# nv-tlabs/LION

Measured on AMD Instinct MI355X. Metric: shapes/sec @1000-step DDIM, Bx2048pts, higher is better.
Workload: dtype f32 (operands of the 3x3x3 voxel convolutions and of the long 1x1 convolutions cut into fp16 hi/lo pairs on the 16-bi...

## Files before the change

lion_amd/csrc/conv3d_split.hip:

```cpp
#include "conv3d_split_kernel.h"

namespace {

__global__ void split_pack_kernel(const float *__restrict__ w, int Cout, int Cin, unsigned short *__restrict__ wp,
                                  unsigned *__restrict__ tail) {
  const int i = blockIdx.x * blockDim.x + threadIdx.x;
  const int ew = split_tail_scale(tail, i == 0);
  if (i >= Cout * Cin * 27) return;
  const int t = i % 27, c = (i / 27) % Cin, co = i / (27 * Cin), chunk = c / KS, g = (c % KS) / 8, j = c % 8;
  unsigned short hi, lo;
  cut(w[i] * pow2f(ew), hi, lo);
  const size_t base = ((size_t)chunk * 27 + t) * 4;
  wp[((base + 0 + g) * Cout + co) * 8 + j] = hi;
  wp[((base + 2 + g) * Cout + co) * 8 + j] = lo;
}

template <bool PRO, bool STATS, int NW>
__global__ __launch_bounds__(64 * NW, 1) void conv3d_split_pipe_kernel(const float *__restrict__ x, const u4 *__restrict__ wp,
                                                                  const float *__restrict__ wtail,
                                                                  const float *__restrict__ bias, float *__restrict__ y,
                                                                  int Cin, int Cout, const float *__restrict__ pro_a,
                                                                  const float *__restrict__ pro_b,
                                                                  float *__restrict__ stats) {
  constexpr int r = 8, r3 = 512, TD = 4, TH = 8, TW = 8, VB = 8 / NW, COT = 32, TM = 64 * NW;
  static_assert(NW == 4 || NW == 8, "4 waves x 2 column blocks or 8 waves x 1");
  constexpr int HD = TD + 2, HH = TH + 2, HW = NW == 8 ? TW + 4 : TW + 2, HALO = HD * HH * HW;
  constexpr int HP = (HALO + 63) / 64 * 64;
  constexpr int WPL = 4 * COT, TG = 9, NG = 27 / TG;
  constexpr int DMA_PER_GROUP = TG * WPL / 64, DMA_MIN = DMA_PER_GROUP / NW;
  extern __shared__ __attribute__((aligned(16))) unsigned char smem[];
  u4 *sx = reinterpret_cast<u4 *>(smem);
  u4 *sw = sx + 2 * 4 * HP;
  float *sbias = reinterpret_cast<float *>(sw + 3 * TG * WPL);
  const int npro = PRO ? ((Cin + 63) & ~63) : 0;
  float *spa = sbias + COT, *spb = spa + npro;
  float *sred = spb + npro;
  __shared__ unsigned s_max[2];
  const int tid = threadIdx.x, lane = tid & 63, wave = __builtin_amdgcn_readfirstlane(tid >> 6);
  const int g = lane >> 5, l32 = lane & 31;
  const int b = blockIdx.x, tile = blockIdx.y, co0 = blockIdx.z * COT, d0 = tile * TD;
  const float wscale_inv = wtail[2];
  if (PRO)
    for (int c = tid; c < Cin; c += TM) { spa[c] = pro_a[(size_t)b * Cin + c]; spb[c] = pro_b[(size_t)b * Cin + c]; }
  if (tid < COT) sbias[tid] = bias ? bias[co0 + tid] : 0.f;
  if (tid < 2) s_max[tid] = 0u;
  int E = 127;

  static_assert(NW == 8, "the quad staging is laid out for 512 threads");
  constexpr int NLOAD = 4;
  const int st_ig = tid / 192, st_u = tid % 192, st_ch4 = st_u / 96, st_rq = st_u % 96;
  const int st_row = st_rq >> 1, st_quad = st_rq & 1, st_hd = st_row >> 3, st_gh = st_row & 7;
  const int st_gd = d0 - 1 + st_hd;
  const bool gok = tid < 384 && st_gd >= 0 && st_gd < r;
  const int goff = gok ? ((st_gd * r + st_gh) * r + st_quad * 4) * 4 + (st_ig * 8 + st_ch4 * 4) * r3 * 4 : 0x7fffff00;
  const int st_pos = (st_hd * HH + st_gh + 1) * HW + st_quad * 4 + 1;
  const __amdgpu_buffer_rsrc_t xrs = __builtin_amdgcn_make_buffer_rsrc(
      const_cast<float *>(x + (size_t)b * Cin * r3), 0, Cin * r3 * 4, 0x00020000);
  int xbase[VB], vox[VB];
#pragma unroll
  for (int vb = 0; vb < VB; ++vb) {
    const int vbk = wave * VB + vb;
    const int d = vbk >> 1, w = l32 & 7;
    const int h = NW == 8 ? (vbk & 1) + 2 * (l32 >> 3) : (vbk & 1) * 2 + ((l32 >> 4) & 1) + 4 * ((l32 >> 3) & 1);
    xbase[vb] = (d * HH + h) * HW + w;
    vox[vb] = ((d0 + d) * r + h) * r + w;
  }
  f32x16 acc[VB], cor[VB], cor2[VB];
#pragma unroll
  for (int vb = 0; vb < VB; ++vb)
#pragma unroll
    for (int i = 0; i < 16; ++i) acc[vb][i] = cor[vb][i] = cor2[vb][i] = 0.f;

  const int nchunks = Cin / KS, ngroups = nchunks * NG;
  typedef __attribute__((address_space(3))) unsigned char lds_byte;
  const uint32_t sw_lds = (uint32_t)(uintptr_t)(lds_byte *)reinterpret_cast<unsigned char *>(sw);
  auto weights_dma = [&](int sg) {
    const u4 *src = wp + (size_t)sg * TG * 4 * Cout + co0;
    const uint32_t dst0 = sw_lds + (uint32_t)((sg % 3) * TG * WPL * 16);
    for (int i = wave; i < DMA_PER_GROUP; i += NW) {
      const u4 *gp = src + (size_t)((i >> 1) * 4 + (i & 1) * 2 + g) * Cout + l32;
      const uint32_t dst = __builtin_amdgcn_readfirstlane(dst0 + (uint32_t)(i * 1024));
      unsigned keep;
      asm volatile("s_mov_b32 %0, m0\n\ts_mov_b32 m0, %2\n\ts_nop 0\n\tglobal_load_lds_dwordx4 %1, off\n\ts_mov_b32 m0, %0"
                   : "=&s"(keep) : "v"(gp), "s"(dst) : "memory");
    }
  };
  typedef float f4 __attribute__((ext_vector_type(4)));
  f4 v[NLOAD];
  auto issue_loads = [&](int q) {
#pragma unroll
    for (int j = 0; j < NLOAD; ++j)
      v[j] = __builtin_bit_cast(f4, __builtin_amdgcn_raw_buffer_load_b128(xrs, goff, (q * KS + j) * r3 * 4, 0));
  };
  auto stage = [&](int q) {
    unsigned mloc = 0u;
    if (PRO) {
      const int c0 = q * KS + st_ig * 8 + st_ch4 * 4;
      const float4 a4 = *reinterpret_cast<const float4 *>(spa + (tid < 384 ? c0 : 0));
      const float4 b4 = *reinterpret_cast<const float4 *>(spb + (tid < 384 ? c0 : 0));
      const float pa[4] = {a4.x, a4.y, a4.z, a4.w}, pb[4] = {b4.x, b4.y, b4.z, b4.w};
#pragma unroll
      for (int j = 0; j < NLOAD; ++j)
#pragma unroll
        for (int k = 0; k < 4; ++k) {
          const float act = pro_act(v[j][k], pa[j], pb[j]);
          v[j][k] = gok ? act : 0.f;
        }
    }
#pragma unroll
    for (int j = 0; j < NLOAD; ++j)
#pragma unroll
      for (int k = 0; k < 4; ++k) {
        const unsigned a = __float_as_uint(v[j][k]) & 0x7fffffffu;
        mloc = (a > mloc && a <= 0x7f7fffffu) ? a : mloc;
      }
    mloc = wave_max_u32_lane63(mloc);
    if (lane == 63 && mloc) atomicMax(&s_max[q & 1], mloc);
    __syncthreads();
    const unsigned mbits = s_max[q & 1];
    if (tid == 0) s_max[(q + 1) & 1] = 0u;
    if (mbits) {
      const int e = scale_exp(__uint_as_float(mbits));
      if (e < E) {
        if (E != 127) {
          const float f = pow2f(max(e - CONV_SPLIT_HEADROOM - E, -126));
#pragma unroll
          for (int vb = 0; vb < VB; ++vb)
#pragma unroll
            for (int i = 0; i < 16; ++i) { acc[vb][i] *= f; cor[vb][i] *= f; cor2[vb][i] *= f; }
        }
        E = e - CONV_SPLIT_HEADROOM;
      }
    }
    const float xs = E == 127 ? 1.0f : pow2f(E);
    if (tid < 384) {
      uint2 *dst2 = reinterpret_cast<uint2 *>(sx + (q & 1) * 4 * HP);
#pragma unroll
      for (int k = 0; k < 4; ++k) {
        unsigned h0, l0, h1, l1;
        cut2(v[0][k] * xs, v[1][k] * xs, h0, l0);
        cut2(v[2][k] * xs, v[3][k] * xs, h1, l1);
        dst2[((0 + st_ig) * HP + st_pos + k) * 2 + st_ch4] = make_uint2(h0, h1);
        dst2[((2 + st_ig) * HP + st_pos + k) * 2 + st_ch4] = make_uint2(l0, l1);
      }
    }
  };

  for (int e = tid; e < 2 * 4 * HP; e += TM) sx[e] = u4{0u, 0u, 0u, 0u};
  weights_dma(0);
  if (ngroups > 1) weights_dma(1);
  issue_loads(0);
  __syncthreads();
  stage(0);
  for (int q = 0; q < nchunks; ++q) {
    const u4 *sxq = sx + (q & 1) * 4 * HP;
    const bool more = q + 1 < nchunks;
#pragma unroll
    for (int grp = 0; grp < NG; ++grp) {
      const int sg = q * NG + grp;
      const bool dma_behind = sg + 1 < ngroups;
      if (grp == 0 || !more) { if (dma_behind) wait_vm<DMA_MIN>(); else wait_vm<0>(); }
      else { if (dma_behind) wait_vm<DMA_MIN + NLOAD>(); else wait_vm<NLOAD>(); }
      __syncthreads();
      if (sg + 2 < ngroups) weights_dma(sg + 2);
      if (grp == 0 && more) issue_loads(q + 1);
      const u4 *swg = sw + (sg % 3) * TG * WPL;
      u4 wf[2][2], xf[2][VB][2];
      auto frags = [&](int t, int s_) {
        const int tap = grp * TG + t;
        const int toff = ((tap / 9) * HH + (tap / 3) % 3) * HW + tap % 3;
#pragma unroll
        for (int pc = 0; pc < 2; ++pc) {
          wf[s_][pc] = swg[t * WPL + (pc * 2 + g) * COT + l32];
#pragma unroll
          for (int vb = 0; vb < VB; ++vb) xf[s_][vb][pc] = sxq[(pc * 2 + g) * HP + xbase[vb] + toff];
        }
      };
      frags(0, 0);
#pragma unroll
      for (int t = 0; t < TG; ++t) {
        if (t + 1 < TG) frags(t + 1, (t + 1) & 1);
        __builtin_amdgcn_sched_barrier(0);
#pragma unroll
        for (int vb = 0; vb < VB; ++vb) {
          acc[vb] = mma(wf[t & 1][0], xf[t & 1][vb][0], acc[vb]);
          cor[vb] = mma(wf[t & 1][0], xf[t & 1][vb][1], cor[vb]);
          cor2[vb] = mma(wf[t & 1][1], xf[t & 1][vb][0], cor2[vb]);
        }
        __builtin_amdgcn_sched_barrier(0);
      }
    }
    if (more) stage(q + 1);
  }

  float *yb = y + ((size_t)b * Cout + co0) * r3;
  const float us_x = E == 127 ? 1.0f : pow2f(-E), us_w = wscale_inv;
#pragma unroll
  for (int vb = 0; vb < VB; ++vb)
#pragma unroll
    for (int i = 0; i < 16; ++i) {
      const int co = (i & 3) + 8 * (i >> 2) + 4 * g;
      const float o = ((acc[vb][i] + (cor[vb][i] + cor2[vb][i]) * (1.f / 2048.f)) * us_x) * us_w + sbias[co];
      acc[vb][i] = o;
      yb[(size_t)co * r3 + vox[vb]] = o;
    }
  if (STATS) {
#pragma unroll
    for (int i = 0; i < 16; ++i) {
      float s1 = acc[0][i], s2 = acc[0][i] * acc[0][i];
#pragma unroll
      for (int vb = 1; vb < VB; ++vb) { s1 += acc[vb][i]; s2 += acc[vb][i] * acc[vb][i]; }
      s1 = row16_sum_rn(s1); s2 = row16_sum_rn(s2);
      s1 = row_pair_sum_odd_rows(s1); s2 = row_pair_sum_odd_rows(s2);
      if (l32 == 16) {
        const int co = (i & 3) + 8 * (i >> 2) + 4 * g;
        sred[(wave * COT + co) * 2] = s1;
        sred[(wave * COT + co) * 2 + 1] = s2;
      }
    }
    __syncthreads();
    if (tid < COT) {
      float s1 = 0.f, s2 = 0.f;
#pragma unroll
      for (int w = 0; w < NW; ++w) { s1 += sred[(w * COT + tid) * 2]; s2 += sred[(w * COT + tid) * 2 + 1]; }
      float *o = stats + (((size_t)b * Cout + co0 + tid) * (r / TD) + tile) * 2;
      o[0] = s1;
      o[1] = s2;
    }
  }
}

template <int NW>
static int launch_split_pipe(const float *x, const u4 *wp, const float *wtail, const float *bias, float *y, int B, int Cin,
                             int Cout, const float *pa, const float *pb, float *stats, hipStream_t st) {
  constexpr int HP = NW == 8 ? 768 : 640, COT = 32;
  const dim3 grid(B, 2, Cout / COT);
  const size_t LDS = (size_t)(2 * 4 * HP + 3 * 9 * 4 * COT) * 16 +
                     (size_t)(COT + (pa ? 2 * ((Cin + 63) & ~63) : 0) + NW * COT * 2) * 4;
#define LION_PIPE_GO(PRO_, ST_)                                                                              \
  {                                                                                                          \
    static LionLdsLimit cfg = {};                                                                            \
    if (int e = lion_dynamic_lds(&conv3d_split_pipe_kernel<PRO_, ST_, NW>, LDS, cfg)) return e;              \
    conv3d_split_pipe_kernel<PRO_, ST_, NW><<<grid, 64 * NW, LDS, st>>>(x, wp, wtail, bias, y, Cin, Cout, pa, pb, stats); \
  }
  if (pa && stats) LION_PIPE_GO(true, true)
  else if (pa) LION_PIPE_GO(true, false)
  else if (stats) LION_PIPE_GO(false, true)
  else LION_PIPE_GO(false, false)
#undef LION_PIPE_GO
  LION_LAUNCH_CHECK();
  return 0;
}

struct SplitPlan { int vb, cb, tiles; };
static SplitPlan split_plan(int r, int Cout) {
  const int r3 = r * r * r;
  const int cb = Cout % 64 == 0 ? 2 : Cout % 32 == 0 ? 1 : 0;
  if (r == 8) return {2, Cout % 32 == 0 ? 1 : 0, 2};
  return {2, cb, r3 / 256};
}

}

extern "C" {

size_t lion_conv3d_split_packed_halfs(int Cout, int Cin) { return split_piece_halfs(Cout, Cin) + 8; }

int lion_conv3d_split_pack_weights(const float *w, int Cout, int Cin, uint16_t *wp, lionStream_t stream) {
  if (!w || !wp || Cout <= 0 || Cin <= 0) return LION_EINVAL;
  if (Cin % KS != 0 || (((uintptr_t)wp) & 15) != 0) return LION_EUNSUPPORTED;
  hipStream_t st = static_cast<hipStream_t>(stream);
  unsigned *tail = reinterpret_cast<unsigned *>(wp + split_piece_halfs(Cout, Cin));
  const int n = Cout * Cin * 27;
  if (hipMemsetAsync(tail, 0, 16, st) != hipSuccess) return LION_EINVAL;
  split_wmax_kernel<<<min(lion_cdiv(n, 2048), 128), 256, 0, st>>>(w, n, tail);
  split_pack_kernel<<<lion_cdiv(n, 256), 256, 0, st>>>(w, Cout, Cin, wp, tail);
  LION_LAUNCH_CHECK();
  return 0;
}


int lion_conv3d_split_stat_tiles(int r, int Cout) {
  if (r != 8 && r != 16 && r != 32) return 0;
  return split_plan(r, Cout).tiles;
}

int lion_conv3d_k3_split_forward(const float *x, const uint16_t *wp, const float *bias, int B, int Cin, int Cout,
                                 int r, const float *pro_a, const float *pro_b, const float *pro_bias,
                                 const float *tconst, float *y, float *stats, int32_t *occ, lionStream_t stream) {
  if (!x || !wp || !y || B <= 0 || Cin <= 0 || Cout <= 0) return LION_EINVAL;
  if ((pro_a == nullptr) != (pro_b == nullptr)) return LION_EINVAL;
  if (tconst && !pro_a) return LION_EINVAL;
  if (occ && pro_a && !tconst) return LION_EINVAL;
  if (Cin % KS != 0 || (pro_a && Cin > 256)) return LION_EUNSUPPORTED;
  if (r != 8 && r != 16 && r != 32) return LION_EUNSUPPORTED;
  if (occ && r == 8) return LION_EUNSUPPORTED;
  const SplitPlan p = split_plan(r, Cout);
  if (!p.cb) return LION_EUNSUPPORTED;
  hipStream_t st = static_cast<hipStream_t>(stream);
  const u4 *w4 = reinterpret_cast<const u4 *>(wp);
  const float *wtail = reinterpret_cast<const float *>(wp + split_piece_halfs(Cout, Cin));
  if (r == 8) {
    if (tconst) return LION_EUNSUPPORTED;
    return launch_split_pipe<8>(x, w4, wtail, bias, y, B, Cin, Cout, pro_a, pro_b, stats, st);
  }
#define LION_SPLIT_TILE(R_, VB_, CB_, TD_, TH_, TW_, OCC_)                                                  \
  if (r == R_ && p.vb == VB_ && p.cb == CB_)                                                                \
    return launch_split_t<TD_, TH_, TW_, CB_, VB_, OCC_, 2>(x, w4, wtail, bias, y, B, Cin, Cout, r, pro_a, pro_b, pro_bias, tconst, \
                                                   stats, occ, st);
  LION_SPLIT_TILE(32, 2, 2, 2, 4, 32, 2)
  LION_SPLIT_TILE(32, 2, 1, 2, 4, 32, 2)
  LION_SPLIT_TILE(16, 2, 2, 4, 4, 16, 2)
  LION_SPLIT_TILE(16, 2, 1, 4, 4, 16, 2)
#undef LION_SPLIT_TILE
  return LION_EUNSUPPORTED;
}

}
```

Baseline: 5.378.

## Interleave next-chunk staging into r=8 conv MMA loop behind env toggle

Adds an OVL template mode to the r=8 voxel conv pipeline kernel. The next chunk's activation, max reduction, rescale and hi/lo cut-and-store are sliced across the tap loop of the current chunk's MMA groups, so they no longer run as a serial stage between chunks. The initial DMA and loads are also issued before the LDS zero-fill. The NW template is removed and the kernel is hardwired to 8 waves. The mode is on by default and can be disabled with LION_CONV_R8_OVERLAP=0. It risks extra register pressure and schedule interference with the MMA stream, and the s_max reset timing changes.

```diff
diff --git a/lion_amd/csrc/conv3d_split.hip b/lion_amd/csrc/conv3d_split.hip
--- a/lion_amd/csrc/conv3d_split.hip
+++ b/lion_amd/csrc/conv3d_split.hip
@@ -15,16 +15,15 @@
   wp[((base + 2 + g) * Cout + co) * 8 + j] = lo;
 }
 
-template <bool PRO, bool STATS, int NW>
-__global__ __launch_bounds__(64 * NW, 1) void conv3d_split_pipe_kernel(const float *__restrict__ x, const u4 *__restrict__ wp,
-                                                                  const float *__restrict__ wtail,
-                                                                  const float *__restrict__ bias, float *__restrict__ y,
-                                                                  int Cin, int Cout, const float *__restrict__ pro_a,
-                                                                  const float *__restrict__ pro_b,
-                                                                  float *__restrict__ stats) {
-  constexpr int r = 8, r3 = 512, TD = 4, TH = 8, TW = 8, VB = 8 / NW, COT = 32, TM = 64 * NW;
-  static_assert(NW == 4 || NW == 8, "4 waves x 2 column blocks or 8 waves x 1");
-  constexpr int HD = TD + 2, HH = TH + 2, HW = NW == 8 ? TW + 4 : TW + 2, HALO = HD * HH * HW;
+template <bool PRO, bool STATS, bool OVL>
+__global__ __launch_bounds__(512, 1) void conv3d_split_pipe_kernel(const float *__restrict__ x, const u4 *__restrict__ wp,
+                                                                 const float *__restrict__ wtail,
+                                                                 const float *__restrict__ bias, float *__restrict__ y,
+                                                                 int Cin, int Cout, const float *__restrict__ pro_a,
+                                                                 const float *__restrict__ pro_b,
+                                                                 float *__restrict__ stats) {
+  constexpr int NW = 8, r = 8, r3 = 512, TD = 4, TH = 8, TW = 8, COT = 32, TM = 64 * NW;
+  constexpr int HD = TD + 2, HH = TH + 2, HW = TW + 4, HALO = HD * HH * HW;
   constexpr int HP = (HALO + 63) / 64 * 64;
   constexpr int WPL = 4 * COT, TG = 9, NG = 27 / TG;
   constexpr int DMA_PER_GROUP = TG * WPL / 64, DMA_MIN = DMA_PER_GROUP / NW;
@@ -46,7 +45,6 @@
   if (tid < 2) s_max[tid] = 0u;
   int E = 127;
 
-  static_assert(NW == 8, "the quad staging is laid out for 512 threads");
   constexpr int NLOAD = 4;
   const int st_ig = tid / 192, st_u = tid % 192, st_ch4 = st_u / 96, st_rq = st_u % 96;
   const int st_row = st_rq >> 1, st_quad = st_rq & 1, st_hd = st_row >> 3, st_gh = st_row & 7;
@@ -56,20 +54,11 @@
   const int st_pos = (st_hd * HH + st_gh + 1) * HW + st_quad * 4 + 1;
   const __amdgpu_buffer_rsrc_t xrs = __builtin_amdgcn_make_buffer_rsrc(
       const_cast<float *>(x + (size_t)b * Cin * r3), 0, Cin * r3 * 4, 0x00020000);
-  int xbase[VB], vox[VB];
-#pragma unroll
-  for (int vb = 0; vb < VB; ++vb) {
-    const int vbk = wave * VB + vb;
-    const int d = vbk >> 1, w = l32 & 7;
-    const int h = NW == 8 ? (vbk & 1) + 2 * (l32 >> 3) : (vbk & 1) * 2 + ((l32 >> 4) & 1) + 4 * ((l32 >> 3) & 1);
-    xbase[vb] = (d * HH + h) * HW + w;
-    vox[vb] = ((d0 + d) * r + h) * r + w;
-  }
-  f32x16 acc[VB], cor[VB], cor2[VB];
-#pragma unroll
-  for (int vb = 0; vb < VB; ++vb)
-#pragma unroll
-    for (int i = 0; i < 16; ++i) acc[vb][i] = cor[vb][i] = cor2[vb][i] = 0.f;
+  const int vd = wave >> 1, vw = l32 & 7, vh = (wave & 1) + 2 * (l32 >> 3);
+  const int xbase = (vd * HH + vh) * HW + vw, vox = ((d0 + vd) * r + vh) * r + vw;
+  f32x16 acc, cor, cor2;
+#pragma unroll
+  for (int i = 0; i < 16; ++i) acc[i] = cor[i] = cor2[i] = 0.f;
 
   const int nchunks = Cin / KS, ngroups = nchunks * NG;
   typedef __attribute__((address_space(3))) unsigned char lds_byte;
@@ -92,69 +81,97 @@
     for (int j = 0; j < NLOAD; ++j)
       v[j] = __builtin_bit_cast(f4, __builtin_amdgcn_raw_buffer_load_b128(xrs, goff, (q * KS + j) * r3 * 4, 0));
   };
+  float pa[NLOAD], pb[NLOAD];
+  auto pro_scalars = [&](int q) {
+    const int c0 = q * KS + st_ig * 8 + st_ch4 * 4;
+    const float4 a4 = *reinterpret_cast<const float4 *>(spa + (tid < 384 ? c0 : 0));
+    const float4 b4 = *reinterpret_cast<const float4 *>(spb + (tid < 384 ? c0 : 0));
+    pa[0] = a4.x; pa[1] = a4.y; pa[2] = a4.z; pa[3] = a4.w;
+    pb[0] = b4.x; pb[1] = b4.y; pb[2] = b4.z; pb[3] = b4.w;
+  };
+  auto activate = [&](int j, int k) {
+    const float act = pro_act(v[j][k], pa[j], pb[j]);
+    v[j][k] = gok ? act : 0.f;
+  };
+  auto finite_max = [&](unsigned m, int j, int k) {
+    const unsigned a = __float_as_uint(v[j][k]) & 0x7fffffffu;
+    return (a > m && a <= 0x7f7fffffu) ? a : m;
+  };
+  auto publish_max = [&](unsigned m, int q) {
+    m = wave_max_u32_lane63(m);
+    if (lane == 63 && m) atomicMax(&s_max[q & 1], m);
+  };
+  auto next_scale = [&](unsigned mbits) {
+    if (mbits) {
+      const int e = scale_exp(__uint_as_float(mbits));
+      if (e < E) return e - CONV_SPLIT_HEADROOM;
+    }
+    return E;
+  };
+  auto rescale_to = [&](int En) {
+    if (En != E) {
+      if (E != 127) {
+        const float f = pow2f(max(En - E, -126));
+#pragma unroll
+        for (int i = 0; i < 16; ++i) { acc[i] *= f; cor[i] *= f; cor2[i] *= f; }
+      }
+      E = En;
+    }
+  };
+  auto cut_store = [&](int q, int k, float xs) {
+    if (tid < 384) {
+      uint2 *dst2 = reinterpret_cast<uint2 *>(sx + (q & 1) * 4 * HP);
+      unsigned h0, l0, h1, l1;
+      cut2(v[0][k] * xs, v[1][k] * xs, h0, l0);
+      cut2(v[2][k] * xs, v[3][k] * xs, h1, l1);
+      dst2[((0 + st_ig) * HP + st_pos + k) * 2 + st_ch4] = make_uint2(h0, h1);
+      dst2[((2 + st_ig) * HP + st_pos + k) * 2 + st_ch4] = make_uint2(l0, l1);
+    }
+  };
   auto stage = [&](int q) {
     unsigned mloc = 0u;
     if (PRO) {
-      const int c0 = q * KS + st_ig * 8 + st_ch4 * 4;
-      const float4 a4 = *reinterpret_cast<const float4 *>(spa + (tid < 384 ? c0 : 0));
-      const float4 b4 = *reinterpret_cast<const float4 *>(spb + (tid < 384 ? c0 : 0));
-      const float pa[4] = {a4.x, a4.y, a4.z, a4.w}, pb[4] = {b4.x, b4.y, b4.z, b4.w};
+      pro_scalars(q);
 #pragma unroll
       for (int j = 0; j < NLOAD; ++j)
 #pragma unroll
-        for (int k = 0; k < 4; ++k) {
-          const float act = pro_act(v[j][k], pa[j], pb[j]);
-          v[j][k] = gok ? act : 0.f;
-        }
+        for (int k = 0; k < 4; ++k) activate(j, k);
     }
 #pragma unroll
     for (int j = 0; j < NLOAD; ++j)
 #pragma unroll
-      for (int k = 0; k < 4; ++k) {
-        const unsigned a = __float_as_uint(v[j][k]) & 0x7fffffffu;
-        mloc = (a > mloc && a <= 0x7f7fffffu) ? a : mloc;
-      }
-    mloc = wave_max_u32_lane63(mloc);
-    if (lane == 63 && mloc) atomicMax(&s_max[q & 1], mloc);
+      for (int k = 0; k < 4; ++k) mloc = finite_max(mloc, j, k);
+    publish_max(mloc, q);
     __syncthreads();
     const unsigned mbits = s_max[q & 1];
-    if (tid == 0) s_max[(q + 1) & 1] = 0u;
-    if (mbits) {
-      const int e = scale_exp(__uint_as_float(mbits));
-      if (e < E) {
-        if (E != 127) {
-          const float f = pow2f(max(e - CONV_SPLIT_HEADROOM - E, -126));
-#pragma unroll
-          for (int vb = 0; vb < VB; ++vb)
-#pragma unroll
-            for (int i = 0; i < 16; ++i) { acc[vb][i] *= f; cor[vb][i] *= f; cor2[vb][i] *= f; }
-        }
-        E = e - CONV_SPLIT_HEADROOM;
-      }
-    }
+    if (!OVL && tid == 0) s_max[(q + 1) & 1] = 0u;
+    rescale_to(next_scale(mbits));
     const float xs = E == 127 ? 1.0f : pow2f(E);
-    if (tid < 384) {
-      uint2 *dst2 = reinterpret_cast<uint2 *>(sx + (q & 1) * 4 * HP);
-#pragma unroll
-      for (int k = 0; k < 4; ++k) {
-        unsigned h0, l0, h1, l1;
-        cut2(v[0][k] * xs, v[1][k] * xs, h0, l0);
-        cut2(v[2][k] * xs, v[3][k] * xs, h1, l1);
-        dst2[((0 + st_ig) * HP + st_pos + k) * 2 + st_ch4] = make_uint2(h0, h1);
-        dst2[((2 + st_ig) * HP + st_pos + k) * 2 + st_ch4] = make_uint2(l0, l1);
-      }
-    }
-  };
-
+#pragma unroll
+    for (int k = 0; k < 4; ++k) cut_store(q, k, xs);
+  };
+
+  if (OVL) {
+    weights_dma(0);
+    if (ngroups > 1) weights_dma(1);
+    issue_loads(0);
+  }
   for (int e = tid; e < 2 * 4 * HP; e += TM) sx[e] = u4{0u, 0u, 0u, 0u};
-  weights_dma(0);
-  if (ngroups > 1) weights_dma(1);
-  issue_loads(0);
+  if (!OVL) {
+    weights_dma(0);
+    if (ngroups > 1) weights_dma(1);
+    issue_loads(0);
+  }
   __syncthreads();
+  if (OVL) __builtin_amdgcn_sched_barrier(0);
   stage(0);
-  for (int q = 0; q < nchunks; ++q) {
+  auto chunk = [&](int q, auto more_c) {
+    constexpr bool SLICE = OVL && decltype(more_c)::value;
+    const bool more = OVL ? SLICE : q + 1 < nchunks;
     const u4 *sxq = sx + (q & 1) * 4 * HP;
-    const bool more = q + 1 < nchunks;
+    unsigned mloc = 0u;
+    int E_next = E;
+    float xs_next = 1.0f;
 #pragma unroll
     for (int grp = 0; grp < NG; ++grp) {
       const int sg = q * NG + grp;
@@ -162,54 +179,82 @@
       if (grp == 0 || !more) { if (dma_behind) wait_vm<DMA_MIN>(); else wait_vm<0>(); }
       else { if (dma_behind) wait_vm<DMA_MIN + NLOAD>(); else wait_vm<NLOAD>(); }
       __syncthreads();
+      if (OVL && grp == 0 && tid == 0) s_max[q & 1] = 0u;
       if (sg + 2 < ngroups) weights_dma(sg + 2);
       if (grp == 0 && more) issue_loads(q + 1);
+      if (SLICE) {
+        if (PRO && grp == 1) pro_scalars(q + 1);
+        if (grp == 2) {
+          E_next = next_scale(s_max[(q + 1) & 1]);
+          xs_next = E_next == 127 ? 1.0f : pow2f(E_next);
+        }
+      }
       const u4 *swg = sw + (sg % 3) * TG * WPL;
-      u4 wf[2][2], xf[2][VB][2];
+      u4 wf[2][2], xf[2][2];
       auto frags = [&](int t, int s_) {
         const int tap = grp * TG + t;
         const int toff = ((tap / 9) * HH + (tap / 3) % 3) * HW + tap % 3;
 #pragma unroll
         for (int pc = 0; pc < 2; ++pc) {
           wf[s_][pc] = swg[t * WPL + (pc * 2 + g) * COT + l32];
-#pragma unroll
-          for (int vb = 0; vb < VB; ++vb) xf[s_][vb][pc] = sxq[(pc * 2 + g) * HP + xbase[vb] + toff];
+          xf[s_][pc] = sxq[(pc * 2 + g) * HP + xbase + toff];
         }
       };
       frags(0, 0);
 #pragma unroll
       for (int t = 0; t < TG; ++t) {
+        if (SLICE && grp == 1 && t == 1) wait_vm<DMA_MIN>();
         if (t + 1 < TG) frags(t + 1, (t + 1) & 1);
+        auto slice = [&]() {
+          if (grp == 1 && t >= 1) {
+#pragma unroll
+            for (int i = 2 * (t - 1); i < 2 * t; ++i) {
+              if (PRO) activate(i >> 2, i & 3);
+              mloc = finite_max(mloc, i >> 2, i & 3);
+            }
+          }
+          if (grp == 2 && (t & 1)) cut_store(q + 1, t >> 1, xs_next);
+        };
+        if (SLICE) slice();
         __builtin_amdgcn_sched_barrier(0);
-#pragma unroll
-        for (int vb = 0; vb < VB; ++vb) {
-          acc[vb] = mma(wf[t & 1][0], xf[t & 1][vb][0], acc[vb]);
-          cor[vb] = mma(wf[t & 1][0], xf[t & 1][vb][1], cor[vb]);
-          cor2[vb] = mma(wf[t & 1][1], xf[t & 1][vb][0], cor2[vb]);
+        acc = mma(wf[t & 1][0], xf[t & 1][0], acc);
+        cor = mma(wf[t & 1][0], xf[t & 1][1], cor);
+        cor2 = mma(wf[t & 1][1], xf[t & 1][0], cor2);
+        __builtin_amdgcn_sched_barrier(0);
+      }
+      if (SLICE) {
+        if (grp == 1) {
+          publish_max(mloc, q + 1);
         }
-        __builtin_amdgcn_sched_barrier(0);
-      }
-    }
-    if (more) stage(q + 1);
+        if (grp == 2) {
+          rescale_to(E_next);
+        }
+      }
+    }
+    if (!OVL) {
+      if (more) stage(q + 1);
+    }
+  };
+  if (OVL) {
+    for (int q = 0; q + 1 < nchunks; ++q) chunk(q, BoolC<true>{});
+    chunk(nchunks - 1, BoolC<false>{});
+  } else {
+    for (int q = 0; q < nchunks; ++q) chunk(q, BoolC<false>{});
   }
 
   float *yb = y + ((size_t)b * Cout + co0) * r3;
   const float us_x = E == 127 ? 1.0f : pow2f(-E), us_w = wscale_inv;
 #pragma unroll
-  for (int vb = 0; vb < VB; ++vb)
+  for (int i = 0; i < 16; ++i) {
+    const int co = (i & 3) + 8 * (i >> 2) + 4 * g;
+    const float o = ((acc[i] + (cor[i] + cor2[i]) * (1.f / 2048.f)) * us_x) * us_w + sbias[co];
+    acc[i] = o;
+    yb[(size_t)co * r3 + vox] = o;
+  }
+  if (STATS) {
 #pragma unroll
     for (int i = 0; i < 16; ++i) {
-      const int co = (i & 3) + 8 * (i >> 2) + 4 * g;
-      const float o = ((acc[vb][i] + (cor[vb][i] + cor2[vb][i]) * (1.f / 2048.f)) * us_x) * us_w + sbias[co];
-      acc[vb][i] = o;
-      yb[(size_t)co * r3 + vox[vb]] = o;
-    }
-  if (STATS) {
-#pragma unroll
-    for (int i = 0; i < 16; ++i) {
-      float s1 = acc[0][i], s2 = acc[0][i] * acc[0][i];
-#pragma unroll
-      for (int vb = 1; vb < VB; ++vb) { s1 += acc[vb][i]; s2 += acc[vb][i] * acc[vb][i]; }
+      float s1 = acc[i], s2 = acc[i] * acc[i];
       s1 = row16_sum_rn(s1); s2 = row16_sum_rn(s2);
       s1 = row_pair_sum_odd_rows(s1); s2 = row_pair_sum_odd_rows(s2);
       if (l32 == 16) {
@@ -230,23 +275,30 @@
   }
 }
 
-template <int NW>
 static int launch_split_pipe(const float *x, const u4 *wp, const float *wtail, const float *bias, float *y, int B, int Cin,
                              int Cout, const float *pa, const float *pb, float *stats, hipStream_t st) {
-  constexpr int HP = NW == 8 ? 768 : 640, COT = 32;
+  constexpr int NW = 8, HP = 768, COT = 32;
   const dim3 grid(B, 2, Cout / COT);
   const size_t LDS = (size_t)(2 * 4 * HP + 3 * 9 * 4 * COT) * 16 +
                      (size_t)(COT + (pa ? 2 * ((Cin + 63) & ~63) : 0) + NW * COT * 2) * 4;
-#define LION_PIPE_GO(PRO_, ST_)                                                                              \
+  const char *ovl_env = getenv("LION_CONV_R8_OVERLAP");
+  const bool ovl = !(ovl_env && ovl_env[0] == '0');
+#define LION_PIPE_GO(PRO_, ST_, OVL_)                                                                        \
   {                                                                                                          \
     static LionLdsLimit cfg = {};                                                                            \
-    if (int e = lion_dynamic_lds(&conv3d_split_pipe_kernel<PRO_, ST_, NW>, LDS, cfg)) return e;              \
-    conv3d_split_pipe_kernel<PRO_, ST_, NW><<<grid, 64 * NW, LDS, st>>>(x, wp, wtail, bias, y, Cin, Cout, pa, pb, stats); \
-  }
-  if (pa && stats) LION_PIPE_GO(true, true)
-  else if (pa) LION_PIPE_GO(true, false)
-  else if (stats) LION_PIPE_GO(false, true)
-  else LION_PIPE_GO(false, false)
+    if (int e = lion_dynamic_lds(&conv3d_split_pipe_kernel<PRO_, ST_, OVL_>, LDS, cfg)) return e;            \
+    conv3d_split_pipe_kernel<PRO_, ST_, OVL_><<<grid, 64 * NW, LDS, st>>>(x, wp, wtail, bias, y, Cin, Cout, pa, pb, stats); \
+  }
+#define LION_PIPE_SEL(PRO_, ST_)                                                                             \
+  {                                                                                                          \
+    if (ovl) LION_PIPE_GO(PRO_, ST_, true)                                                                   \
+    else LION_PIPE_GO(PRO_, ST_, false)                                                                      \
+  }
+  if (pa && stats) LION_PIPE_SEL(true, true)
+  else if (pa) LION_PIPE_SEL(true, false)
+  else if (stats) LION_PIPE_SEL(false, true)
+  else LION_PIPE_SEL(false, false)
+#undef LION_PIPE_SEL
 #undef LION_PIPE_GO
   LION_LAUNCH_CHECK();
   return 0;
@@ -302,7 +354,7 @@
   const float *wtail = reinterpret_cast<const float *>(wp + split_piece_halfs(Cout, Cin));
   if (r == 8) {
     if (tconst) return LION_EUNSUPPORTED;
-    return launch_split_pipe<8>(x, w4, wtail, bias, y, B, Cin, Cout, pro_a, pro_b, stats, st);
+    return launch_split_pipe(x, w4, wtail, bias, y, B, Cin, Cout, pro_a, pro_b, stats, st);
   }
 #define LION_SPLIT_TILE(R_, VB_, CB_, TD_, TH_, TW_, OCC_)                                                  \
   if (r == R_ && p.vb == VB_ && p.cb == CB_)                                                                \
```

Measured after the change: 5.409, median of 6. About the same (+0.6%).
